# jiangzhengkai/mxdetection

Measured on AMD Instinct MI355X. Metric: images/sec (whole node) Faster R-CNN R50-FPN 3x800x1333, higher is better.
Workload: dtype bf16; 1 GPU; Faster R-CNN ResNet-50-FPN bf16 train step, batch 2/GPU, 3x800x1333 (padded 1344); global_batch=2, parallelism=dp1, frozen=stem+C2, frozen BN folded, optimizer=SGD momentum 0.9 wd 1e-4, launch=hipGraph replay, input=resident, wgrad_side_stream=True, rpn_branch_stream=True, grouped_wgrad=True, filter_prefetch_hints=True, params_trainable=41538304

## Files before the change

### include/mxdet.h

```cpp
#ifndef MXDET_H_
#define MXDET_H_

#include <stddef.h>
#include <stdint.h>

#ifdef __cplusplus
extern "C" {
#endif

#define MXDET_OK 0
#define MXDET_EINVAL (-1)
#define MXDET_ESHAPE (-2)
#define MXDET_EWORKSPACE (-3)
#define MXDET_EHIP (-4)
#define MXDET_ERCCL (-5)

#define MXDET_DTYPE_F32 0
#define MXDET_DTYPE_BF16 1

typedef void* mxdet_stream_t;

const char* mxdet_last_error(void);
const char* mxdet_version(void);

// ... 85 lines not shown
                         const int32_t* matched_gt, const float* gt_boxes, int32_t N, int32_t G_max, int64_t R,
                         int32_t num_classes, int32_t reg_dim, int32_t kind, float sigma, float std_x, float std_y,
                         float std_w, float std_h, float reg_weight, float* score, mxdet_stream_t stream);
size_t mxdet_ohem_select_workspace_bytes(int32_t N, int32_t P);
int mxdet_ohem_select(const float* score, const int32_t* labels, const float* rois, int32_t N, int32_t P, int32_t R,
                      float nms_thresh, int32_t* sel, int32_t* num_sel, int32_t* num_fg, void* workspace,
                      size_t workspace_bytes, mxdet_stream_t stream);
int mxdet_ohem_gather(const int32_t* sel, const float* pool_rois, const int32_t* pool_labels,
                      const int32_t* pool_matched_gt, const float* pool_bbox_targets, const float* pool_bbox_weights,
                      int32_t N, int32_t P, int32_t R, int32_t reg_dim, float* out_rois, int32_t* labels,
                      float* bbox_targets, float* bbox_weights, int32_t* matched_gt, mxdet_stream_t stream);

int mxdet_fpn_level_map(const float* rois, int64_t R, int32_t lvl_min, int32_t lvl_max,
                        int32_t* levels, mxdet_stream_t stream);
typedef struct {
  int32_t num_levels, lvl_min;
  int32_t H[8], W[8];
  float spatial_scale[8];
  void* feat[8];
} mxdet_feat_pyramid_t;
int mxdet_roi_align_fwd(const mxdet_feat_pyramid_t* f, int32_t N, int32_t C, const float* rois,
                        const int32_t* levels, int64_t R, int32_t PH, int32_t PW,
                        int32_t sampling_ratio, uint16_t* out, mxdet_stream_t stream);
int mxdet_roi_align_bwd(const mxdet_feat_pyramid_t* f, int32_t N, int32_t C, const float* rois,
                        const int32_t* levels, int64_t R, int32_t PH, int32_t PW,
                        int32_t sampling_ratio, const uint16_t* grad_out, mxdet_stream_t stream);
size_t mxdet_roi_align_bwd_gather_workspace_bytes(const mxdet_feat_pyramid_t* f, int32_t N, int64_t R);
int mxdet_roi_align_bwd_gather(const mxdet_feat_pyramid_t* f, int32_t N, int32_t C, const float* rois,
                               const int32_t* levels, int64_t R, int32_t PH, int32_t PW, int32_t sampling_ratio,
                               const uint16_t* grad_out, int32_t accumulate, void* workspace, size_t workspace_bytes,
                               mxdet_stream_t stream);
int mxdet_roi_align_bwd_gather_prepare(const mxdet_feat_pyramid_t* f, int32_t N, const float* rois,
                                       const int32_t* levels, int64_t R, int32_t PH, int32_t PW, int32_t sampling_ratio,
                                       void* workspace, size_t workspace_bytes, mxdet_stream_t stream);
int mxdet_roi_align_bwd_gather_prepared(const mxdet_feat_pyramid_t* f, int32_t N, int32_t C, const float* rois,
                                        const int32_t* levels, int64_t R, int32_t PH, int32_t PW, int32_t sampling_ratio,
                                        const uint16_t* grad_out, int32_t accumulate, void* workspace,
                                        size_t workspace_bytes, mxdet_stream_t stream);

typedef struct {
  mxdet_feat_pyramid_t pyr;
  int32_t N, C;
  int32_t PH, PW;
  int32_t sample_per_part;
  float trans_std;
  int32_t modulated;
// ... 376 lines not shown
```

### mxdetection_amd/_lib.py

```python
import ctypes as C
import os

_HERE = os.path.dirname(os.path.abspath(__file__))
LIB_PATH = os.environ.get("MXDET_LIB") or os.path.join(_HERE, "libmxdet_hip.so")

c_i32, c_i64, c_u32, c_f32, c_sz, c_vp = C.c_int32, C.c_int64, C.c_uint32, C.c_float, C.c_size_t, C.c_void_p


class PyramidT(C.Structure):
    _fields_ = [
        ("num_levels", c_i32), ("A", c_i32),
        ("H", c_i32 * 8), ("W", c_i32 * 8), ("stride", c_i32 * 8),
        ("cls", c_vp * 8), ("reg", c_vp * 8),
        ("cls_sn", c_i64 * 8), ("cls_sy", c_i64 * 8), ("cls_sx", c_i64 * 8), ("cls_sa", c_i64 * 8),
        ("reg_sn", c_i64 * 8), ("reg_sy", c_i64 * 8), ("reg_sx", c_i64 * 8), ("reg_sc", c_i64 * 8),
        ("dtype", c_i32), ("classes", c_i32),
        ("base_anchors", c_vp * 8),
    ]


class FeatPyramidT(C.Structure):
    _fields_ = [
        ("num_levels", c_i32), ("lvl_min", c_i32),
        ("H", c_i32 * 8), ("W", c_i32 * 8),
# ... 107 lines not shown
    "mxdet_proposal": (c_i32, [P(PyramidT), c_i32, c_vp, c_i32, c_i32, c_f32, c_f32, c_vp, c_vp, c_vp, c_vp,
                               c_vp, c_sz, c_vp]),
    "mxdet_anchor_target_workspace_bytes": (c_sz, [c_i32, c_i64, c_i32]),
    "mxdet_anchor_target": (c_i32, [c_vp, c_i64, c_vp, c_i32, c_i32, c_vp, c_f32, c_f32, c_f32, c_i32, c_f32,
                                    c_u32, c_u32, c_vp, c_u32, c_vp, c_vp, c_vp, c_vp, c_vp, c_sz, c_vp]),
    "mxdet_atss_assign_workspace_bytes": (c_sz, [c_i32, c_i64, c_i32]),
    "mxdet_atss_assign": (c_i32, [c_vp, c_i64, P(c_i64), c_i32, c_vp, c_i32, c_i32, c_i32, c_vp, c_vp, c_vp, c_vp, c_vp, c_sz,
                                  c_vp]),
    "mxdet_proposal_target": (c_i32, [c_vp, c_vp, c_i32, c_vp, c_i32, c_i32, c_i32, c_f32, c_f32, c_f32, c_f32,
                                      c_i32, c_i32, P(c_f32), P(c_f32), c_u32, c_u32, c_vp, c_u32, c_vp, c_vp, c_vp,
                                      c_vp, c_vp, c_vp, c_vp]),
    "mxdet_proposal_target_balanced": (c_i32, [c_vp, c_vp, c_i32, c_vp, c_i32, c_i32, c_i32, c_f32, c_f32, c_f32, c_f32,
                                               c_i32, c_i32, P(c_f32), P(c_f32), c_u32, c_u32, c_vp, c_u32, c_i32, c_vp, c_vp,
                                               c_vp, c_vp, c_vp, c_vp, c_vp]),
    "mxdet_ohem_roi_score": (c_i32, [c_vp, c_vp, c_i32, c_i32, c_i32, c_vp, c_vp, c_vp, c_vp, c_vp, c_vp, c_i32, c_i32, c_i64,
                                     c_i32, c_i32, c_i32, c_f32, c_f32, c_f32, c_f32, c_f32, c_f32, c_vp, c_vp]),
    "mxdet_ohem_select_workspace_bytes": (c_sz, [c_i32, c_i32]),
    "mxdet_ohem_select": (c_i32, [c_vp, c_vp, c_vp, c_i32, c_i32, c_i32, c_f32, c_vp, c_vp, c_vp, c_vp, c_sz, c_vp]),
    "mxdet_ohem_gather": (c_i32, [c_vp, c_vp, c_vp, c_vp, c_vp, c_vp, c_i32, c_i32, c_i32, c_i32, c_vp, c_vp, c_vp, c_vp,
                                  c_vp, c_vp]),
    "mxdet_fpn_level_map": (c_i32, [c_vp, c_i64, c_i32, c_i32, c_vp, c_vp]),
    "mxdet_roi_align_fwd": (c_i32, [P(FeatPyramidT), c_i32, c_i32, c_vp, c_vp, c_i64, c_i32, c_i32, c_i32, c_vp,
                                    c_vp]),
    "mxdet_roi_align_bwd": (c_i32, [P(FeatPyramidT), c_i32, c_i32, c_vp, c_vp, c_i64, c_i32, c_i32, c_i32, c_vp,
                                    c_vp]),
    "mxdet_roi_align_bwd_gather_workspace_bytes": (c_sz, [P(FeatPyramidT), c_i32, c_i64]),
    "mxdet_roi_align_bwd_gather": (c_i32, [P(FeatPyramidT), c_i32, c_i32, c_vp, c_vp, c_i64, c_i32, c_i32, c_i32, c_vp,
                                           c_i32, c_vp, c_sz, c_vp]),
    "mxdet_roi_align_bwd_gather_prepare": (c_i32, [P(FeatPyramidT), c_i32, c_vp, c_vp, c_i64, c_i32, c_i32, c_i32,
                                                   c_vp, c_sz, c_vp]),
    "mxdet_roi_align_bwd_gather_prepared": (c_i32, [P(FeatPyramidT), c_i32, c_i32, c_vp, c_vp, c_i64, c_i32, c_i32, c_i32,
                                                    c_vp, c_i32, c_vp, c_sz, c_vp]),
    "mxdet_smooth_l1_fwd": (c_i32, [c_vp, c_vp, c_vp, c_i64, c_f32, c_vp, c_vp]),
    "mxdet_smooth_l1_bwd": (c_i32, [c_vp, c_vp, c_vp, c_vp, c_i64, c_f32, c_i32, c_vp, c_vp]),
    "mxdet_loss_workspace_bytes": (c_sz, [c_i64]),
    "mxdet_focal_loss": (c_i32, [c_vp, c_i32, c_vp, c_i64, c_i32, c_f32, c_f32, c_f32, c_vp, c_vp, c_vp, c_sz,
                                 c_vp]),
    "mxdet_anchor_class_labels": (c_i32, [c_vp, c_vp, c_vp, c_i32, c_i64, c_i32, c_vp, c_vp, c_vp]),
    "mxdet_retina_loss_num_partials": (c_i32, [c_i32, c_i32, c_i32, c_i32]),
    "mxdet_retina_loss_level": (c_i32, [c_vp, c_vp, c_i32, c_i32, c_i32, c_i32, c_i32, c_i32, c_i32, c_vp, c_vp, c_i64,
                                        c_i64, c_f32, c_f32, c_f32, c_vp, c_f32, c_vp, c_vp, c_vp, c_vp]),
    "mxdet_rpn_loss_num_partials": (c_i32, [c_i32, c_i32, c_i32]),
    "mxdet_rpn_loss_level": (c_i32, [c_vp, c_i32, c_i32, c_i32, c_i32, c_i32, c_vp, c_vp, c_i64, c_i64, c_f32,
                                     c_f32, c_f32, c_vp, c_vp, c_vp]),
    "mxdet_loss_finalize": (c_i32, [c_vp, c_i32, c_i32, c_vp, c_vp]),
    "mxdet_rcnn_loss": (c_i32, [c_vp, c_vp, c_i32, c_i32, c_i32, c_vp, c_vp, c_vp, c_i64, c_i32, c_i32, c_f32,
# ... 168 lines not shown
```

### mxdetection_amd/csrc/roi_align.hip

```cpp
#include "roi_gather.h"

namespace mxdet {

struct RoiGeom {
  float start_w, start_h, bin_w, bin_h;
  int gh, gw, H, W, batch, lvl;
};

__device__ __forceinline__ RoiGeom roi_geom(const FeatPyr& f, const float* __restrict__ rois,
                                            const int32_t* __restrict__ levels, long long r, int PH,
                                            int PW, int sampling_ratio) {
  RoiGeom g;
  const float* q = rois + r * 5;
  roi_image_level(f, rois, levels, r, &g.lvl, &g.batch);
  const int l = g.lvl;
  float s = f.scale[l];
  g.start_w = q[1] * s;
  g.start_h = q[2] * s;
  float end_w = q[3] * s, end_h = q[4] * s;
  float rw = end_w - g.start_w, rh = end_h - g.start_h;
  rw = rw > 1.0f ? rw : 1.0f;
  rh = rh > 1.0f ? rh : 1.0f;
  g.bin_h = rh / (float)PH;
  g.bin_w = rw / (float)PW;
  if (sampling_ratio > 0) {
    g.gh = sampling_ratio;
    g.gw = sampling_ratio;
  } else {
    float ch = rh / (float)PH, cw = rw / (float)PW;
    int ih = (int)ch, iw = (int)cw;
    g.gh = ((float)ih < ch) ? ih + 1 : ih;
    g.gw = ((float)iw < cw) ? iw + 1 : iw;
  }
  g.H = f.H[l];
  g.W = f.W[l];
  return g;
}

struct Taps {
  int yl, yh, xl, xh;
  float w1, w2, w3, w4;
  bool valid;
};

__device__ __forceinline__ float roi_sample_coord(float start, float bin, int b, int i, int g) {
  float v = start + (float)b * bin;
  return v + (((float)i + 0.5f) * bin) / (float)g;
}

template <int SR>
__device__ __forceinline__ float roi_axis_coord(float start, float bin, int s, int sr) {
  const int b = SR ? s / SR : s / sr, i = s - b * (SR ? SR : sr);
  return roi_sample_coord(start, bin, b, i, SR ? SR : sr);
}

struct AxisSample { int lo, hi; float wlo, whi; bool valid; };

__device__ __forceinline__ AxisSample roi_axis_sample(float v, int L) {
  AxisSample a;
  a.valid = !(v < -1.0f || v > (float)L);
  if (v <= 0.0f) v = 0.0f;
  int lo = (int)v;
  if (lo >= L - 1) { a.hi = lo = L - 1; v = (float)lo; } else { a.hi = lo + 1; }
  a.lo = lo;
  a.whi = v - (float)lo;
  a.wlo = 1.0f - a.whi;
  return a;
}

__device__ __forceinline__ Taps bilinear_taps(float y, float x, int H, int W) {
  const AxisSample ay = roi_axis_sample(y, H), ax = roi_axis_sample(x, W);
  Taps t;
  t.valid = ay.valid && ax.valid;
  t.w1 = ay.wlo * ax.wlo; t.w2 = ay.wlo * ax.whi; t.w3 = ay.whi * ax.wlo; t.w4 = ay.whi * ax.whi;
  t.yl = ay.lo; t.yh = ay.hi; t.xl = ax.lo; t.xh = ax.hi;
  return t;
}

__global__ void __launch_bounds__(256)
roi_align_fwd_kernel(FeatPyr f, int C, const float* __restrict__ rois,
                     const int32_t* __restrict__ levels, int PH, int PW, int sampling_ratio,
                     uint16_t* __restrict__ out) {
  const long long r = blockIdx.x;
  const RoiGeom g = roi_geom(f, rois, levels, r, PH, PW, sampling_ratio);
  const int CG = C >> 3;
  const int items = PH * PW * CG;
  const uint16_t* feat = (const uint16_t*)f.feat[g.lvl] + (long long)g.batch * g.H * g.W * C;
  const float count = (float)(g.gh * g.gw);
  for (int it = threadIdx.x; it < items; it += blockDim.x) {
    int cg = it % CG;
    int bin = it / CG;
    int pw = bin % PW, ph = bin / PW;
    float acc[8];
#pragma unroll
    for (int k = 0; k < 8; ++k) acc[k] = 0.0f;
    for (int iy = 0; iy < g.gh; ++iy) {
      const float y = roi_sample_coord(g.start_h, g.bin_h, ph, iy, g.gh);
      for (int ix = 0; ix < g.gw; ++ix) {
        const float x = roi_sample_coord(g.start_w, g.bin_w, pw, ix, g.gw);
        const Taps t = bilinear_taps(y, x, g.H, g.W);
        if (!t.valid) continue;
        const uint4 v1 = *(const uint4*)(feat + ((long long)t.yl * g.W + t.xl) * C + cg * 8);
        const uint4 v2 = *(const uint4*)(feat + ((long long)t.yl * g.W + t.xh) * C + cg * 8);
        const uint4 v3 = *(const uint4*)(feat + ((long long)t.yh * g.W + t.xl) * C + cg * 8);
        const uint4 v4 = *(const uint4*)(feat + ((long long)t.yh * g.W + t.xh) * C + cg * 8);
        float a[8], b[8], c[8], d[8];
        unpack8_bf16(v1, a); unpack8_bf16(v2, b); unpack8_bf16(v3, c); unpack8_bf16(v4, d);
#pragma unroll
        for (int k = 0; k < 8; ++k) {
          float s = t.w1 * a[k];
          s = s + t.w2 * b[k];
          s = s + t.w3 * c[k];
          s = s + t.w4 * d[k];
          acc[k] = acc[k] + s;
        }
      }
    }
    uint32_t o[4];
#pragma unroll
    for (int k = 0; k < 4; ++k) {
      uint32_t lo = mxdet_f32_to_bf16(acc[2 * k] / count);
      uint32_t hi = mxdet_f32_to_bf16(acc[2 * k + 1] / count);
      o[k] = lo | (hi << 16);
    }
    *(uint4*)(out + (r * PH * PW + bin) * C + cg * 8) = make_uint4(o[0], o[1], o[2], o[3]);
  }
}

__global__ void __launch_bounds__(256)
roi_align_bwd_kernel(FeatPyr f, int C, const float* __restrict__ rois,
                     const int32_t* __restrict__ levels, int PH, int PW, int sampling_ratio,
                     const uint16_t* __restrict__ gout) {
  const long long r = blockIdx.x;
  const RoiGeom g = roi_geom(f, rois, levels, r, PH, PW, sampling_ratio);
  const int items = PH * PW * C;
  float* dfeat = (float*)f.feat[g.lvl] + (long long)g.batch * g.H * g.W * C;
  const float count = (float)(g.gh * g.gw);
// ... 182 lines not shown
          }
        }
      }
     }
    }
    if (accumulate && !touched) continue;
#pragma unroll
    for (int j = 0; j < kRoiTileW; ++j) {
      if (x0 + j >= W || !live) break;
      const float v[4] = {a0[j], a1[j], a2[j], a3[j]};
      seg_store4<true>(out + (size_t)j * C + c0, v, accumulate);
    }
  }
}

struct RoiSegGrid {
  int block0[9];
  int chunks[8];
  int segs_per_wg[8];
  int rows_per_wg[8];
  int bands[8];
};

struct RoiSeg {
  int nl;
  unsigned yy, xx;
  int r;
  float start_h, bin_h, start_w, bin_w;
};

typedef float f32x2_t __attribute__((ext_vector_type(2)));

__device__ __forceinline__ float lane_plus1(float v) {
  return __uint_as_float((unsigned)__builtin_amdgcn_update_dpp(0, (int)__float_as_uint(v), 0x101, 0xf, 0xf, true));
}

__device__ __forceinline__ void roi_axis_range(float start, float bin, int NS, int sr, int L, int* lo, int* hi) {
  int s0 = 0, s1 = NS - 1;
  while (s0 <= s1 && !roi_axis_sample(roi_axis_coord<0>(start, bin, s0, sr), L).valid) ++s0;
  while (s1 >= s0 && !roi_axis_sample(roi_axis_coord<0>(start, bin, s1, sr), L).valid) --s1;
  if (s0 > s1) { *lo = 1; *hi = 0; return; }
  *lo = roi_axis_sample(roi_axis_coord<0>(start, bin, s0, sr), L).lo;
  *hi = roi_axis_sample(roi_axis_coord<0>(start, bin, s1, sr), L).hi;
}

__global__ void __launch_bounds__(256)
roi_bwd_box_kernel(FeatPyr f, const float* __restrict__ rois, const int32_t* __restrict__ levels, int R, int PH, int PW,
                   int sr, RoiSeg* __restrict__ seg) {
  const int r = (int)(blockIdx.x * blockDim.x + threadIdx.x);
  if (r >= R) return;
  const RoiGeom g = roi_geom(f, rois, levels, r, PH, PW, sr);
  int ylo, yhi, xlo, xhi;
  roi_axis_range(g.start_h, g.bin_h, PH * sr, sr, g.H, &ylo, &yhi);
  roi_axis_range(g.start_w, g.bin_w, PW * sr, sr, g.W, &xlo, &xhi);
  RoiSeg o;
  const bool any = ylo <= yhi && xlo <= xhi;
  o.nl = g.batch | ((any ? g.lvl : 0xffff) << 16);
  o.yy = span_pack(ylo, yhi);
  o.xx = span_pack(xlo, xhi);
  o.r = r;
  o.start_h = g.start_h; o.bin_h = g.bin_h; o.start_w = g.start_w; o.bin_w = g.bin_w;
  seg[r] = o;
}

template <int PWT, int SR>
__global__ void __launch_bounds__(kSegWaves * 64)
roi_bwd_seg_kernel(FeatPyr f, RoiSegGrid gr, int C, const RoiSeg* __restrict__ seg, int R, int PH, int PW, int sr_,
                   const uint16_t* __restrict__ gout, int accumulate) {
  __shared__ unsigned e_xx[kSegChunk], e_yy[kSegChunk];
  __shared__ int e_r[kSegChunk];
  __shared__ float4 e_g[kSegChunk];
  __shared__ int wcnt[kSegWaves];
  __shared__ int s_cnt;
  const int sr = SR ? SR : sr_;
  const int tid = threadIdx.x, lane = tid & 63;
  const int wid = __builtin_amdgcn_readfirstlane(tid >> 6);
  const int bid = (int)blockIdx.x;
  const int l = level_of_block(gr.block0, f.num_levels, bid);
  const int rel = bid - gr.block0[l];
  const int per_img = gr.bands[l] * gr.chunks[l];
  const int n = rel / per_img, rem = rel - n * per_img;
  const int band = rem / gr.chunks[l], chunk = rem - band * gr.chunks[l];
  const int H = f.H[l], W = f.W[l];
  const int Y0 = band * gr.rows_per_wg[l];
  const int Y1 = (Y0 + gr.rows_per_wg[l] - 1 < H - 1) ? Y0 + gr.rows_per_wg[l] - 1 : H - 1;
// ... 133 lines not shown
      if (!live || (!multi_row && !last_round)) continue;
      const bool add = accumulate || (multi_row && !first_round);
      if (add && !touched) continue;
      uint16_t* out = (uint16_t*)f.feat[l] + ((size_t)(n * H + Y) * W + x0) * C + c0;
#pragma unroll
      for (int j = 0; j < kSegW; ++j) {
        if (x0 + j >= W) break;
        const float v[4] = {acc[j][0][0], acc[j][0][1], acc[j][1][0], acc[j][1][1]};
        seg_store4<true>(out + (size_t)j * C, v, add);
      }
    }
  }
}

static int fill(FeatPyr& d, const mxdet_feat_pyramid_t* f, int N, const char* who) {
  MXDET_REQUIRE(f != nullptr, MXDET_EINVAL, "%s: null pyramid", who);
  MXDET_REQUIRE(f->num_levels > 0 && f->num_levels <= 8, MXDET_ESHAPE, "%s: bad level count", who);
  for (int l = 0; l < f->num_levels; ++l)
    MXDET_REQUIRE(f->H[l] > 0 && f->W[l] > 0 && f->feat[l], MXDET_EINVAL, "%s: level %d incomplete", who, l);
  pyr_copy(d, *f, N);
  return MXDET_OK;
}

}

using namespace mxdet;

extern "C" int mxdet_roi_align_fwd(const mxdet_feat_pyramid_t* f, int32_t N, int32_t C,
                                   const float* rois, const int32_t* levels, int64_t R, int32_t PH,
                                   int32_t PW, int32_t sampling_ratio, uint16_t* out,
                                   mxdet_stream_t stream) {
  clear_error();
  FeatPyr d;
  int rc = fill(d, f, N, "roi_align_fwd");
  if (rc) return rc;
  MXDET_REQUIRE(N > 0 && C > 0 && (C % 8) == 0 && PH > 0 && PW > 0 && R >= 0, MXDET_ESHAPE,
                "roi_align_fwd: bad shape (C must be a multiple of 8)");
  if (R == 0) return MXDET_OK;
  MXDET_REQUIRE(rois && levels && out, MXDET_EINVAL, "roi_align_fwd: null pointer");
  hipLaunchKernelGGL(roi_align_fwd_kernel, dim3((unsigned)R), dim3(256), 0, as_stream(stream), d, C,
                     rois, levels, PH, PW, sampling_ratio, out);
  return check_launch("roi_align_fwd");
}

extern "C" int mxdet_roi_align_bwd(const mxdet_feat_pyramid_t* f, int32_t N, int32_t C,
                                   const float* rois, const int32_t* levels, int64_t R, int32_t PH,
                                   int32_t PW, int32_t sampling_ratio, const uint16_t* grad_out,
                                   mxdet_stream_t stream) {
  clear_error();
  FeatPyr d;
  int rc = fill(d, f, N, "roi_align_bwd");
  if (rc) return rc;
  MXDET_REQUIRE(N > 0 && C > 0 && PH > 0 && PW > 0 && R >= 0, MXDET_ESHAPE, "roi_align_bwd: bad shape");
  if (R == 0) return MXDET_OK;
  MXDET_REQUIRE(rois && levels && grad_out, MXDET_EINVAL, "roi_align_bwd: null pointer");
  hipLaunchKernelGGL(roi_align_bwd_kernel, dim3((unsigned)R), dim3(256), 0, as_stream(stream), d, C,
                     rois, levels, PH, PW, sampling_ratio, grad_out);
  return check_launch("roi_align_bwd");
}

static size_t roi_gather_carve(const FeatPyr& d, long long R, RoiRows* rr, size_t* off_tab, size_t* off_list, size_t* off_cnt,
                               size_t* off_box) {
  int rows_of[8], blocks_of[8];
  for (int l = 0; l < d.num_levels; ++l) {
// ... 2 lines not shown
    blocks_of[l] = rows_of[l] * rr->tiles_w[l];
  }
  const int rows = rr->rows_total = layout_block0(rr->row0, rows_of, d.num_levels);
  layout_block0(rr->block0, blocks_of, d.num_levels);
  size_t off = 0;
  *off_tab = off; off = align_up(off + (size_t)R * sizeof(RoiTab), 256);
  *off_list = off; off = align_up(off + (size_t)rows * (size_t)R * sizeof(unsigned short), 256);
  *off_cnt = off; off = align_up(off + (size_t)rows * sizeof(int), 256);
  *off_box = off; off = align_up(off + (size_t)R * sizeof(RoiBox), 256);
  return off;
}

extern "C" size_t mxdet_roi_align_bwd_gather_workspace_bytes(const mxdet_feat_pyramid_t* f, int32_t N, int64_t R) {
  if (!f || N <= 0 || R <= 0 || f->num_levels <= 0 || f->num_levels > 8) return 0;
  FeatPyr d;
  pyr_copy(d, *f, N);
  RoiRows rr; size_t a, b, c, e;
  return roi_gather_carve(d, R, &rr, &a, &b, &c, &e);
}

static int roi_bwd_gather_impl(const mxdet_feat_pyramid_t* f, int32_t N, int32_t C, const float* rois,
                               const int32_t* levels, int64_t R, int32_t PH, int32_t PW,
                               int32_t sampling_ratio, const uint16_t* grad_out, int32_t accumulate,
                               void* workspace, size_t workspace_bytes, mxdet_stream_t stream, int mode) {
  clear_error();
  FeatPyr d;
  int rc = fill(d, f, N, "roi_align_bwd_gather");
  if (rc) return rc;
  MXDET_REQUIRE(N > 0 && C > 0 && (C % 4) == 0 && PH > 0 && PW > 0 && R >= 0, MXDET_ESHAPE, "roi_align_bwd_gather: bad shape (C must be a multiple of 4)");
  MXDET_REQUIRE(sampling_ratio > 0 && PH * sampling_ratio <= kRoiMaxSamples && PW * sampling_ratio <= kRoiMaxSamples,
                MXDET_ESHAPE, "roi_align_bwd_gather: needs 0 < sampling_ratio and at most %d samples per axis", kRoiMaxSamples);
  MXDET_REQUIRE(R <= 65535, MXDET_ESHAPE, "roi_align_bwd_gather: at most 65535 rois");
  for (int l = 0; l < d.num_levels; ++l)
    MXDET_REQUIRE(d.H[l] < 32768 && d.W[l] < 32768, MXDET_ESHAPE, "roi_align_bwd_gather: level %d too large", l);
  MXDET_REQUIRE(rois && levels && (grad_out || mode == 1), MXDET_EINVAL, "roi_align_bwd_gather: null pointer");
  hipStream_t s = as_stream(stream);
  RoiRows rr; size_t o_tab, o_list, o_cnt, o_box;
  const size_t need = roi_gather_carve(d, R > 0 ? R : 1, &rr, &o_tab, &o_list, &o_cnt, &o_box);
  MXDET_REQUIRE(workspace && workspace_bytes >= need, MXDET_EWORKSPACE, "roi_align_bwd_gather: workspace %zu < %zu",
                workspace_bytes, need);
  if (PW <= 14 && R > 0 && tuning(MXDET_TUNE_ROI_TABLE) == 0) {
    static_assert(sizeof(RoiSeg) == sizeof(RoiBox), "the records live in the table form's box array");
    RoiSeg* seg = (RoiSeg*)((char*)workspace + o_box);
    RoiSegGrid gr;
    memset(&gr, 0, sizeof(gr));
    int blocks_of[8];
    const int rows_big = (int)tuning(MXDET_TUNE_ROI_ROWS);
    for (int l = 0; l < d.num_levels; ++l) {
      const int segs = ceil_div(d.W[l], kSegW);
      gr.chunks[l] = ceil_div(segs, kSegWaves);
      gr.segs_per_wg[l] = ceil_div(segs, gr.chunks[l]);
      gr.rows_per_wg[l] = (R > kSegChunk || d.H[l] < 64 || rows_big < 1) ? 1 : rows_big;
      gr.bands[l] = ceil_div(d.H[l], gr.rows_per_wg[l]);
      blocks_of[l] = d.N * gr.bands[l] * gr.chunks[l];
    }
    const int blocks = layout_block0(gr.block0, blocks_of, d.num_levels);
    if (mode != 2)
      hipLaunchKernelGGL(roi_bwd_box_kernel, dim3((unsigned)ceil_div((int)R, 256)), dim3(256), 0, s, d, rois, levels, (int)R,
                         PH, PW, sampling_ratio, seg);
    if (mode == 1) return check_launch("roi_align_bwd_gather_prepare");
    const dim3 grid((unsigned)blocks, (unsigned)ceil_div(C, 256));
#define MXDET_ROI_SEG(PWT, SR)                                                                                          \
  hipLaunchKernelGGL((roi_bwd_seg_kernel<PWT, SR>), grid, dim3(kSegWaves * 64), 0, s, d, gr, C, (const RoiSeg*)seg, (int)R, \
                     PH, PW, sampling_ratio, grad_out, accumulate)
    if (PW <= 7) { if (sampling_ratio == 2) MXDET_ROI_SEG(7, 2); else MXDET_ROI_SEG(7, 0); }
    else { if (sampling_ratio == 2) MXDET_ROI_SEG(14, 2); else MXDET_ROI_SEG(14, 0); }
#undef MXDET_ROI_SEG
    return check_launch("roi_align_bwd_gather");
  }
  if (mode == 1) return MXDET_OK;
  RoiTab* tab = (RoiTab*)((char*)workspace + o_tab);
  unsigned short* list = (unsigned short*)((char*)workspace + o_list);
  int* cnt = (int*)((char*)workspace + o_cnt);
  RoiBox* box = (RoiBox*)((char*)workspace + o_box);
  if (R > 0)
    hipLaunchKernelGGL(roi_bwd_tab_kernel, dim3((unsigned)R), dim3(64), 0, s, d, rois, levels, (long long)R, PH, PW,
                       sampling_ratio, tab, box);
  hipLaunchKernelGGL(roi_bwd_rows_kernel, dim3(rr.rows_total), dim3(64), 0, s, d, rr, (const RoiBox*)box,
                     (int)R, list, cnt);
  hipLaunchKernelGGL(roi_align_bwd_gather_kernel, dim3((unsigned)rr.block0[d.num_levels]), dim3(64), 0, s, d, rr, C,
                     (const RoiTab*)tab, (const RoiBox*)box, (int)R, (const unsigned short*)list, (const int*)cnt, PH, PW,
                     sampling_ratio, grad_out, accumulate);
  return check_launch("roi_align_bwd_gather");
}

extern "C" int mxdet_roi_align_bwd_gather(const mxdet_feat_pyramid_t* f, int32_t N, int32_t C, const float* rois,
                                          const int32_t* levels, int64_t R, int32_t PH, int32_t PW,
                                          int32_t sampling_ratio, const uint16_t* grad_out, int32_t accumulate,
                                          void* workspace, size_t workspace_bytes, mxdet_stream_t stream) {
  return roi_bwd_gather_impl(f, N, C, rois, levels, R, PH, PW, sampling_ratio, grad_out, accumulate, workspace,
                             workspace_bytes, stream, 0);
}

extern "C" int mxdet_roi_align_bwd_gather_prepare(const mxdet_feat_pyramid_t* f, int32_t N, const float* rois,
                                                  const int32_t* levels, int64_t R, int32_t PH, int32_t PW,
                                                  int32_t sampling_ratio, void* workspace, size_t workspace_bytes,
                                                  mxdet_stream_t stream) {
  return roi_bwd_gather_impl(f, N, 4, rois, levels, R, PH, PW, sampling_ratio, nullptr, 0, workspace, workspace_bytes,
                             stream, 1);
}

extern "C" int mxdet_roi_align_bwd_gather_prepared(const mxdet_feat_pyramid_t* f, int32_t N, int32_t C, const float* rois,
                                                   const int32_t* levels, int64_t R, int32_t PH, int32_t PW,
                                                   int32_t sampling_ratio, const uint16_t* grad_out, int32_t accumulate,
                                                   void* workspace, size_t workspace_bytes, mxdet_stream_t stream) {
  return roi_bwd_gather_impl(f, N, C, rois, levels, R, PH, PW, sampling_ratio, grad_out, accumulate, workspace,
                             workspace_bytes, stream, 2);
}
```

### mxdetection_amd/csrc/roi_gather.h

```cpp
#pragma once
#include "common.h"

namespace mxdet {

struct FeatPyr {
  int num_levels, lvl_min, N;
  int H[8], W[8];
  float scale[8];
  void* feat[8];
};

static inline void pyr_copy(FeatPyr& d, const mxdet_feat_pyramid_t& f, int N) {
  memset(&d, 0, sizeof(d));
  d.num_levels = f.num_levels;
  d.lvl_min = f.lvl_min;
  d.N = N;
  for (int l = 0; l < f.num_levels; ++l) {
    d.H[l] = f.H[l]; d.W[l] = f.W[l]; d.scale[l] = f.spatial_scale[l]; d.feat[l] = f.feat[l];
  }
}

__device__ __forceinline__ void roi_image_level(const FeatPyr& f, const float* __restrict__ rois,
                                                const int32_t* __restrict__ levels, long long r, int* lvl, int* n) {
  int l = levels[r] - f.lvl_min;
  *lvl = l < 0 ? 0 : (l >= f.num_levels ? f.num_levels - 1 : l);
  const int b = (int)rois[r * 5];
  *n = b < 0 ? 0 : (b >= f.N ? f.N - 1 : b);
}

static inline int layout_block0(int* block0, const int* per_level, int num_levels) {
  int blocks = 0;
  for (int l = 0; l < num_levels; ++l) {
    block0[l] = blocks;
    blocks += per_level[l];
  }
  block0[num_levels] = blocks;
  return blocks;
}

__device__ __forceinline__ int level_of_block(const int* block0, int num_levels, int bid) {
  int l = 0;
  while (l + 1 < num_levels && bid >= block0[l + 1]) ++l;
  return l;
}

constexpr unsigned kSpanEmpty = 0xffffu;
__device__ __forceinline__ unsigned span_pack(int lo, int hi) { return (unsigned)lo | ((unsigned)hi << 16); }
__device__ __forceinline__ int span_lo(unsigned packed) { return (int)(packed & 0xffffu); }
__device__ __forceinline__ int span_hi(unsigned packed) { return (int)(packed >> 16); }
__device__ __forceinline__ bool span_hits(unsigned packed, int lo, int hi) {
// ... 50 lines not shown
```

### mxdetection_amd/models/roi_extractors/fpn_roi_extractor.py

```python
import torch

from ...ops import dense
from ...ops.roi_align import (fpn_level_map, roi_align_backward, roi_align_backward_gather,
                              roi_align_backward_gather_prepare, roi_align_backward_gather_workspace, roi_align_forward)


class FPNRoIExtractor:
    def __init__(self, strides, pooled=(7, 7), sampling_ratio=2, lvl_min=2, device="cuda"):
        self.scales = [1.0 / s for s in strides]
        self.pooled, self.sr, self.lvl_min = pooled, sampling_ratio, lvl_min
        self.lvl_max = lvl_min + len(strides) - 1
        self.device = device
        self.out = None
        self.outs = {}
        self.dacc = None
        self.gather_ws = {}
        self.prepared = None

    def forward(self, feats, rois, prepare_gather=False):
        self.feats, self.rois = feats[:len(self.scales)], rois
        self.levels = fpn_level_map(rois, self.lvl_min, self.lvl_max)
        R, C = rois.shape[0], feats[0].shape[3]
        self.out = self.outs.setdefault((R, C), None)
        if self.out is None:
            self.out = torch.empty((R, self.pooled[0], self.pooled[1], C), dtype=torch.bfloat16, device=self.device)
            self.outs[(R, C)] = self.out
        self.prepared = None
        if prepare_gather:
            key = (R,) + tuple(tuple(f.shape[:3]) for f in self.feats)
            ws = self.gather_ws.get(key)
            if ws is None:
                ws = self.gather_ws[key] = roi_align_backward_gather_workspace(self.feats, self.scales, R, self.lvl_min)
            roi_align_backward_gather_prepare(self.feats, self.scales, rois, self.levels, self.pooled, self.sr,
                                              self.lvl_min, ws)
            self.prepared = ws
        return roi_align_forward(self.feats, self.scales, rois, self.levels, self.pooled, self.sr, self.lvl_min, self.out)

    def backward(self, grad_out, dP, shared_acc=None, zero=True, finalize=True):
        if shared_acc is not None:
            self.dacc = shared_acc
        if self.dacc is None:
            sizes = [f.numel() for f in self.feats]
            self.dacc_flat = torch.empty((sum(sizes),), dtype=torch.float32, device=self.device)
            self.dacc, off = [], 0
            for f, n in zip(self.feats, sizes):
                self.dacc.append(self.dacc_flat[off:off + n].view(f.shape))
                off += n
        if zero:
            if getattr(self, "dacc_flat", None) is not None:
                self.dacc_flat.zero_()
            else:
                for a in self.dacc:
                    a.zero_()
        roi_align_backward(self.dacc, self.scales, self.rois, self.levels, grad_out, self.sr, self.lvl_min)
        if finalize:
            self.finalize(dP)
        return self.dacc

# ... 15 lines not shown
```

### mxdetection_amd/ops/roi_align.py

```python
import ctypes as C

import torch

from .. import _lib
from .._lib import FeatPyramidT, check, ptr, stream_ptr


def fpn_level_map(rois, lvl_min=2, lvl_max=5):
    lib = _lib.load()
    R = rois.shape[0]
    levels = torch.empty((R,), dtype=torch.int32, device=rois.device)
    check(lib.mxdet_fpn_level_map(ptr(rois), R, lvl_min, lvl_max, ptr(levels), stream_ptr()), "fpn_level_map")
    return levels


def _pyr(feats, scales, lvl_min):
    d = FeatPyramidT()
    d.num_levels, d.lvl_min = len(feats), lvl_min
    for l, f in enumerate(feats):
        d.H[l], d.W[l] = f.shape[1], f.shape[2]
        d.spatial_scale[l] = scales[l]
        d.feat[l] = f.data_ptr()
    return d


def roi_align_forward(feats, scales, rois, levels, pooled=(7, 7), sampling_ratio=2, lvl_min=2, out=None):
    lib = _lib.load()
    N, C_ = feats[0].shape[0], feats[0].shape[3]
    R = rois.shape[0]
    if out is None:
        out = torch.empty((R, pooled[0], pooled[1], C_), dtype=torch.bfloat16, device=rois.device)
    d = _pyr(feats, scales, lvl_min)
    check(lib.mxdet_roi_align_fwd(C.byref(d), N, C_, ptr(rois), ptr(levels), R, pooled[0], pooled[1], sampling_ratio,
                                  ptr(out), stream_ptr()), "roi_align_fwd")
    return out


def roi_align_backward(dfeats, scales, rois, levels, grad_out, sampling_ratio=2, lvl_min=2):
    lib = _lib.load()
    N, C_ = dfeats[0].shape[0], dfeats[0].shape[3]
    R, PH, PW = grad_out.shape[0], grad_out.shape[1], grad_out.shape[2]
    d = _pyr(dfeats, scales, lvl_min)
    check(lib.mxdet_roi_align_bwd(C.byref(d), N, C_, ptr(rois), ptr(levels), R, PH, PW, sampling_ratio,
                                  ptr(grad_out), stream_ptr()), "roi_align_bwd")


_gather_ws = {}


def _gather_workspace(lib, d, N, R, device, workspace):
    need = lib.mxdet_roi_align_bwd_gather_workspace_bytes(C.byref(d), N, R)
    if workspace is None:
        key = (device, need)
        workspace = _gather_ws.get(key)
        if workspace is None:
            workspace = torch.empty((max(need, 256),), dtype=torch.uint8, device=device)
            _gather_ws[key] = workspace
    return workspace
# ... 30 lines not shown
```

Before: 457.3 images/sec.

## Fuse FPN level mapping and backward-gather prep into RoIAlign forward for training

Adds a training RoIAlign forward kernel that works out each RoI's FPN level inline, writes the levels array, and emits the backward-gather segment records from one thread per block. This replaces the separate fpn_level_map and gather-prepare launches. The forward kernel also gains a sampling_ratio=2 specialization that fully unrolls the four samples and issues all tap loads before accumulating, and its launch bounds now request higher occupancy. The cost is more registers per thread from the batched loads and a larger template kernel.

After: 459.6 images/sec (median of 6 runs). About the same (+0.5%).

```diff
diff --git a/include/mxdet.h b/include/mxdet.h
--- a/include/mxdet.h
+++ b/include/mxdet.h
@@ -131,6 +131,9 @@
 int mxdet_roi_align_fwd(const mxdet_feat_pyramid_t* f, int32_t N, int32_t C, const float* rois,
                         const int32_t* levels, int64_t R, int32_t PH, int32_t PW,
                         int32_t sampling_ratio, uint16_t* out, mxdet_stream_t stream);
+int mxdet_roi_align_fwd_train(const mxdet_feat_pyramid_t* f, int32_t N, int32_t C, const float* rois, int64_t R,
+                              int32_t PH, int32_t PW, int32_t sampling_ratio, uint16_t* out, int32_t* levels,
+                              void* workspace, size_t workspace_bytes, mxdet_stream_t stream);
 int mxdet_roi_align_bwd(const mxdet_feat_pyramid_t* f, int32_t N, int32_t C, const float* rois,
                         const int32_t* levels, int64_t R, int32_t PH, int32_t PW,
                         int32_t sampling_ratio, const uint16_t* grad_out, mxdet_stream_t stream);
diff --git a/mxdetection_amd/_lib.py b/mxdetection_amd/_lib.py
--- a/mxdetection_amd/_lib.py
+++ b/mxdetection_amd/_lib.py
@@ -153,6 +153,8 @@
     "mxdet_fpn_level_map": (c_i32, [c_vp, c_i64, c_i32, c_i32, c_vp, c_vp]),
     "mxdet_roi_align_fwd": (c_i32, [P(FeatPyramidT), c_i32, c_i32, c_vp, c_vp, c_i64, c_i32, c_i32, c_i32, c_vp,
                                     c_vp]),
+    "mxdet_roi_align_fwd_train": (c_i32, [P(FeatPyramidT), c_i32, c_i32, c_vp, c_i64, c_i32, c_i32, c_i32, c_vp, c_vp,
+                                          c_vp, c_sz, c_vp]),
     "mxdet_roi_align_bwd": (c_i32, [P(FeatPyramidT), c_i32, c_i32, c_vp, c_vp, c_i64, c_i32, c_i32, c_i32, c_vp,
                                     c_vp]),
     "mxdet_roi_align_bwd_gather_workspace_bytes": (c_sz, [P(FeatPyramidT), c_i32, c_i64]),
diff --git a/mxdetection_amd/csrc/roi_align.hip b/mxdetection_amd/csrc/roi_align.hip
--- a/mxdetection_amd/csrc/roi_align.hip
+++ b/mxdetection_amd/csrc/roi_align.hip
@@ -7,13 +7,12 @@
   int gh, gw, H, W, batch, lvl;
 };
 
-__device__ __forceinline__ RoiGeom roi_geom(const FeatPyr& f, const float* __restrict__ rois,
-                                            const int32_t* __restrict__ levels, long long r, int PH,
-                                            int PW, int sampling_ratio) {
+__device__ __forceinline__ RoiGeom roi_geom_on(const FeatPyr& f, const float* __restrict__ rois, long long r, int l,
+                                               int batch, int PH, int PW, int sampling_ratio) {
   RoiGeom g;
   const float* q = rois + r * 5;
-  roi_image_level(f, rois, levels, r, &g.lvl, &g.batch);
-  const int l = g.lvl;
+  g.lvl = l;
+  g.batch = batch;
   float s = f.scale[l];
   g.start_w = q[1] * s;
   g.start_h = q[2] * s;
@@ -37,6 +36,14 @@
   return g;
 }
 
+__device__ __forceinline__ RoiGeom roi_geom(const FeatPyr& f, const float* __restrict__ rois,
+                                            const int32_t* __restrict__ levels, long long r, int PH,
+                                            int PW, int sampling_ratio) {
+  int l, batch;
+  roi_image_level(f, rois, levels, r, &l, &batch);
+  return roi_geom_on(f, rois, r, l, batch, PH, PW, sampling_ratio);
+}
+
 struct Taps {
   int yl, yh, xl, xh;
   float w1, w2, w3, w4;
@@ -77,12 +84,56 @@
   return t;
 }
 
-__global__ void __launch_bounds__(256)
-roi_align_fwd_kernel(FeatPyr f, int C, const float* __restrict__ rois,
-                     const int32_t* __restrict__ levels, int PH, int PW, int sampling_ratio,
+struct RoiSeg {
+  int nl;
+  unsigned yy, xx;
+  int r;
+  float start_h, bin_h, start_w, bin_w;
+};
+
+__device__ __forceinline__ void roi_axis_range(float start, float bin, int NS, int sr, int L, int* lo, int* hi) {
+  int s0 = 0, s1 = NS - 1;
+  while (s0 <= s1 && !roi_axis_sample(roi_axis_coord<0>(start, bin, s0, sr), L).valid) ++s0;
+  while (s1 >= s0 && !roi_axis_sample(roi_axis_coord<0>(start, bin, s1, sr), L).valid) --s1;
+  if (s0 > s1) { *lo = 1; *hi = 0; return; }
+  *lo = roi_axis_sample(roi_axis_coord<0>(start, bin, s0, sr), L).lo;
+  *hi = roi_axis_sample(roi_axis_coord<0>(start, bin, s1, sr), L).hi;
+}
+
+__device__ __forceinline__ RoiSeg roi_seg_record(const RoiGeom& g, int r, int PH, int PW, int sr) {
+  int ylo, yhi, xlo, xhi;
+  roi_axis_range(g.start_h, g.bin_h, PH * sr, sr, g.H, &ylo, &yhi);
+  roi_axis_range(g.start_w, g.bin_w, PW * sr, sr, g.W, &xlo, &xhi);
+  RoiSeg o;
+  const bool any = ylo <= yhi && xlo <= xhi;
+  o.nl = g.batch | ((any ? g.lvl : 0xffff) << 16);
+  o.yy = span_pack(ylo, yhi);
+  o.xx = span_pack(xlo, xhi);
+  o.r = r;
+  o.start_h = g.start_h; o.bin_h = g.bin_h; o.start_w = g.start_w; o.bin_w = g.bin_w;
+  return o;
+}
+
+template <int SR, bool FUSED>
+__global__ void __launch_bounds__(256, 4)
+roi_align_fwd_kernel(FeatPyr f, int C, const float* __restrict__ rois, const int32_t* __restrict__ levels,
+                     int32_t* __restrict__ levels_out, RoiSeg* __restrict__ seg, int PH, int PW, int sampling_ratio,
                      uint16_t* __restrict__ out) {
   const long long r = blockIdx.x;
-  const RoiGeom g = roi_geom(f, rois, levels, r, PH, PW, sampling_ratio);
+  RoiGeom g;
+  if (FUSED) {
+    const float* q = rois + r * 5;
+    const int lvl_max = f.lvl_min + f.num_levels - 1;
+    int k = mxdet_fpn_level(q[1], q[2], q[3], q[4]);
+    k = k < f.lvl_min ? f.lvl_min : (k > lvl_max ? lvl_max : k);
+    g = roi_geom_on(f, rois, r, k - f.lvl_min, roi_image(f, rois, r), PH, PW, SR ? SR : sampling_ratio);
+    if (threadIdx.x == blockDim.x - 1) {
+      levels_out[r] = k;
+      if (seg) seg[r] = roi_seg_record(g, (int)r, PH, PW, SR ? SR : sampling_ratio);
+    }
+  } else {
+    g = roi_geom(f, rois, levels, r, PH, PW, SR ? SR : sampling_ratio);
+  }
   const int CG = C >> 3;
   const int items = PH * PW * CG;
   const uint16_t* feat = (const uint16_t*)f.feat[g.lvl] + (long long)g.batch * g.H * g.W * C;
@@ -94,25 +145,58 @@
     float acc[8];
 #pragma unroll
     for (int k = 0; k < 8; ++k) acc[k] = 0.0f;
-    for (int iy = 0; iy < g.gh; ++iy) {
-      const float y = roi_sample_coord(g.start_h, g.bin_h, ph, iy, g.gh);
-      for (int ix = 0; ix < g.gw; ++ix) {
-        const float x = roi_sample_coord(g.start_w, g.bin_w, pw, ix, g.gw);
-        const Taps t = bilinear_taps(y, x, g.H, g.W);
-        if (!t.valid) continue;
-        const uint4 v1 = *(const uint4*)(feat + ((long long)t.yl * g.W + t.xl) * C + cg * 8);
-        const uint4 v2 = *(const uint4*)(feat + ((long long)t.yl * g.W + t.xh) * C + cg * 8);
-        const uint4 v3 = *(const uint4*)(feat + ((long long)t.yh * g.W + t.xl) * C + cg * 8);
-        const uint4 v4 = *(const uint4*)(feat + ((long long)t.yh * g.W + t.xh) * C + cg * 8);
+    if (SR) {
+      constexpr int NS = SR ? SR * SR : 1;
+      Taps t[NS];
+#pragma unroll
+      for (int iy = 0; iy < SR; ++iy) {
+        const float y = roi_sample_coord(g.start_h, g.bin_h, ph, iy, SR);
+#pragma unroll
+        for (int ix = 0; ix < SR; ++ix)
+          t[iy * SR + ix] = bilinear_taps(y, roi_sample_coord(g.start_w, g.bin_w, pw, ix, SR), g.H, g.W);
+      }
+      uint4 v[NS][4];
+#pragma unroll
+      for (int s = 0; s < NS; ++s) {
+        v[s][0] = *(const uint4*)(feat + ((long long)t[s].yl * g.W + t[s].xl) * C + cg * 8);
+        v[s][1] = *(const uint4*)(feat + ((long long)t[s].yl * g.W + t[s].xh) * C + cg * 8);
+        v[s][2] = *(const uint4*)(feat + ((long long)t[s].yh * g.W + t[s].xl) * C + cg * 8);
+        v[s][3] = *(const uint4*)(feat + ((long long)t[s].yh * g.W + t[s].xh) * C + cg * 8);
+      }
+#pragma unroll
+      for (int s = 0; s < NS; ++s) {
         float a[8], b[8], c[8], d[8];
-        unpack8_bf16(v1, a); unpack8_bf16(v2, b); unpack8_bf16(v3, c); unpack8_bf16(v4, d);
+        unpack8_bf16(v[s][0], a); unpack8_bf16(v[s][1], b); unpack8_bf16(v[s][2], c); unpack8_bf16(v[s][3], d);
 #pragma unroll
         for (int k = 0; k < 8; ++k) {
-          float s = t.w1 * a[k];
-          s = s + t.w2 * b[k];
-          s = s + t.w3 * c[k];
-          s = s + t.w4 * d[k];
-          acc[k] = acc[k] + s;
+          float u = t[s].w1 * a[k];
+          u = u + t[s].w2 * b[k];
+          u = u + t[s].w3 * c[k];
+          u = u + t[s].w4 * d[k];
+          acc[k] = t[s].valid ? acc[k] + u : acc[k];
+        }
+      }
+    } else {
+      for (int iy = 0; iy < g.gh; ++iy) {
+        const float y = roi_sample_coord(g.start_h, g.bin_h, ph, iy, g.gh);
+        for (int ix = 0; ix < g.gw; ++ix) {
+          const float x = roi_sample_coord(g.start_w, g.bin_w, pw, ix, g.gw);
+          const Taps t = bilinear_taps(y, x, g.H, g.W);
+          if (!t.valid) continue;
+          const uint4 v1 = *(const uint4*)(feat + ((long long)t.yl * g.W + t.xl) * C + cg * 8);
+          const uint4 v2 = *(const uint4*)(feat + ((long long)t.yl * g.W + t.xh) * C + cg * 8);
+          const uint4 v3 = *(const uint4*)(feat + ((long long)t.yh * g.W + t.xl) * C + cg * 8);
+          const uint4 v4 = *(const uint4*)(feat + ((long long)t.yh * g.W + t.xh) * C + cg * 8);
+          float a[8], b[8], c[8], d[8];
+          unpack8_bf16(v1, a); unpack8_bf16(v2, b); unpack8_bf16(v3, c); unpack8_bf16(v4, d);
+#pragma unroll
+          for (int k = 0; k < 8; ++k) {
+            float s = t.w1 * a[k];
+            s = s + t.w2 * b[k];
+            s = s + t.w3 * c[k];
+            s = s + t.w4 * d[k];
+            acc[k] = acc[k] + s;
+          }
         }
       }
     }
@@ -341,26 +425,10 @@
   int bands[8];
 };
 
-struct RoiSeg {
-  int nl;
-  unsigned yy, xx;
-  int r;
-  float start_h, bin_h, start_w, bin_w;
-};
-
 typedef float f32x2_t __attribute__((ext_vector_type(2)));
 
 __device__ __forceinline__ float lane_plus1(float v) {
   return __uint_as_float((unsigned)__builtin_amdgcn_update_dpp(0, (int)__float_as_uint(v), 0x101, 0xf, 0xf, true));
-}
-
-__device__ __forceinline__ void roi_axis_range(float start, float bin, int NS, int sr, int L, int* lo, int* hi) {
-  int s0 = 0, s1 = NS - 1;
-  while (s0 <= s1 && !roi_axis_sample(roi_axis_coord<0>(start, bin, s0, sr), L).valid) ++s0;
-  while (s1 >= s0 && !roi_axis_sample(roi_axis_coord<0>(start, bin, s1, sr), L).valid) --s1;
-  if (s0 > s1) { *lo = 1; *hi = 0; return; }
-  *lo = roi_axis_sample(roi_axis_coord<0>(start, bin, s0, sr), L).lo;
-  *hi = roi_axis_sample(roi_axis_coord<0>(start, bin, s1, sr), L).hi;
 }
 
 __global__ void __launch_bounds__(256)
@@ -368,18 +436,7 @@
                    int sr, RoiSeg* __restrict__ seg) {
   const int r = (int)(blockIdx.x * blockDim.x + threadIdx.x);
   if (r >= R) return;
-  const RoiGeom g = roi_geom(f, rois, levels, r, PH, PW, sr);
-  int ylo, yhi, xlo, xhi;
-  roi_axis_range(g.start_h, g.bin_h, PH * sr, sr, g.H, &ylo, &yhi);
-  roi_axis_range(g.start_w, g.bin_w, PW * sr, sr, g.W, &xlo, &xhi);
-  RoiSeg o;
-  const bool any = ylo <= yhi && xlo <= xhi;
-  o.nl = g.batch | ((any ? g.lvl : 0xffff) << 16);
-  o.yy = span_pack(ylo, yhi);
-  o.xx = span_pack(xlo, xhi);
-  o.r = r;
-  o.start_h = g.start_h; o.bin_h = g.bin_h; o.start_w = g.start_w; o.bin_w = g.bin_w;
-  seg[r] = o;
+  seg[r] = roi_seg_record(roi_geom(f, rois, levels, r, PH, PW, sr), r, PH, PW, sr);
 }
 
 template <int PWT, int SR>
@@ -559,6 +616,17 @@
   return MXDET_OK;
 }
 
+template <bool FUSED>
+static void roi_fwd_launch(const FeatPyr& d, int C, const float* rois, const int32_t* levels, int32_t* levels_out,
+                           RoiSeg* seg, int64_t R, int PH, int PW, int sampling_ratio, uint16_t* out, hipStream_t s) {
+  if (sampling_ratio == 2)
+    hipLaunchKernelGGL((roi_align_fwd_kernel<2, FUSED>), dim3((unsigned)R), dim3(256), 0, s, d, C, rois, levels, levels_out,
+                       seg, PH, PW, sampling_ratio, out);
+  else
+    hipLaunchKernelGGL((roi_align_fwd_kernel<0, FUSED>), dim3((unsigned)R), dim3(256), 0, s, d, C, rois, levels, levels_out,
+                       seg, PH, PW, sampling_ratio, out);
+}
+
 }
 
 using namespace mxdet;
@@ -575,8 +643,7 @@
                 "roi_align_fwd: bad shape (C must be a multiple of 8)");
   if (R == 0) return MXDET_OK;
   MXDET_REQUIRE(rois && levels && out, MXDET_EINVAL, "roi_align_fwd: null pointer");
-  hipLaunchKernelGGL(roi_align_fwd_kernel, dim3((unsigned)R), dim3(256), 0, as_stream(stream), d, C,
-                     rois, levels, PH, PW, sampling_ratio, out);
+  roi_fwd_launch<false>(d, C, rois, levels, nullptr, nullptr, R, PH, PW, sampling_ratio, out, as_stream(stream));
   return check_launch("roi_align_fwd");
 }
 
@@ -625,7 +692,8 @@
 static int roi_bwd_gather_impl(const mxdet_feat_pyramid_t* f, int32_t N, int32_t C, const float* rois,
                                const int32_t* levels, int64_t R, int32_t PH, int32_t PW,
                                int32_t sampling_ratio, const uint16_t* grad_out, int32_t accumulate,
-                               void* workspace, size_t workspace_bytes, mxdet_stream_t stream, int mode) {
+                               void* workspace, size_t workspace_bytes, mxdet_stream_t stream, int mode,
+                               RoiSeg** records = nullptr) {
   clear_error();
   FeatPyr d;
   int rc = fill(d, f, N, "roi_align_bwd_gather");
@@ -636,7 +704,7 @@
   MXDET_REQUIRE(R <= 65535, MXDET_ESHAPE, "roi_align_bwd_gather: at most 65535 rois");
   for (int l = 0; l < d.num_levels; ++l)
     MXDET_REQUIRE(d.H[l] < 32768 && d.W[l] < 32768, MXDET_ESHAPE, "roi_align_bwd_gather: level %d too large", l);
-  MXDET_REQUIRE(rois && levels && (grad_out || mode == 1), MXDET_EINVAL, "roi_align_bwd_gather: null pointer");
+  MXDET_REQUIRE(rois && levels && (grad_out || mode == 1 || mode == 3), MXDET_EINVAL, "roi_align_bwd_gather: null pointer");
   hipStream_t s = as_stream(stream);
   RoiRows rr; size_t o_tab, o_list, o_cnt, o_box;
   const size_t need = roi_gather_carve(d, R > 0 ? R : 1, &rr, &o_tab, &o_list, &o_cnt, &o_box);
@@ -645,6 +713,7 @@
   if (PW <= 14 && R > 0 && tuning(MXDET_TUNE_ROI_TABLE) == 0) {
     static_assert(sizeof(RoiSeg) == sizeof(RoiBox), "the records live in the table form's box array");
     RoiSeg* seg = (RoiSeg*)((char*)workspace + o_box);
+    if (mode == 3) { *records = seg; return MXDET_OK; }
     RoiSegGrid gr;
     memset(&gr, 0, sizeof(gr));
     int blocks_of[8];
@@ -671,7 +740,7 @@
 #undef MXDET_ROI_SEG
     return check_launch("roi_align_bwd_gather");
   }
-  if (mode == 1) return MXDET_OK;
+  if (mode == 1 || mode == 3) return MXDET_OK;
   RoiTab* tab = (RoiTab*)((char*)workspace + o_tab);
   unsigned short* list = (unsigned short*)((char*)workspace + o_list);
   int* cnt = (int*)((char*)workspace + o_cnt);
@@ -710,3 +779,24 @@
   return roi_bwd_gather_impl(f, N, C, rois, levels, R, PH, PW, sampling_ratio, grad_out, accumulate, workspace,
                              workspace_bytes, stream, 2);
 }
+
+extern "C" int mxdet_roi_align_fwd_train(const mxdet_feat_pyramid_t* f, int32_t N, int32_t C, const float* rois, int64_t R,
+                                         int32_t PH, int32_t PW, int32_t sampling_ratio, uint16_t* out, int32_t* levels,
+                                         void* workspace, size_t workspace_bytes, mxdet_stream_t stream) {
+  clear_error();
+  FeatPyr d;
+  int rc = fill(d, f, N, "roi_align_fwd_train");
+  if (rc) return rc;
+  MXDET_REQUIRE(N > 0 && C > 0 && (C % 8) == 0 && PH > 0 && PW > 0 && R >= 0, MXDET_ESHAPE,
+                "roi_align_fwd_train: bad shape (C must be a multiple of 8)");
+  if (R == 0) return MXDET_OK;
+  MXDET_REQUIRE(rois && levels && out, MXDET_EINVAL, "roi_align_fwd_train: null pointer");
+  RoiSeg* seg = nullptr;
+  if (workspace) {
+    rc = roi_bwd_gather_impl(f, N, C, rois, levels, R, PH, PW, sampling_ratio, nullptr, 0, workspace, workspace_bytes,
+                             stream, 3, &seg);
+    if (rc) return rc;
+  }
+  roi_fwd_launch<true>(d, C, rois, nullptr, levels, seg, R, PH, PW, sampling_ratio, out, as_stream(stream));
+  return check_launch("roi_align_fwd_train");
+}
diff --git a/mxdetection_amd/csrc/roi_gather.h b/mxdetection_amd/csrc/roi_gather.h
--- a/mxdetection_amd/csrc/roi_gather.h
+++ b/mxdetection_amd/csrc/roi_gather.h
@@ -20,12 +20,16 @@
   }
 }
 
+__device__ __forceinline__ int roi_image(const FeatPyr& f, const float* __restrict__ rois, long long r) {
+  const int b = (int)rois[r * 5];
+  return b < 0 ? 0 : (b >= f.N ? f.N - 1 : b);
+}
+
 __device__ __forceinline__ void roi_image_level(const FeatPyr& f, const float* __restrict__ rois,
                                                 const int32_t* __restrict__ levels, long long r, int* lvl, int* n) {
   int l = levels[r] - f.lvl_min;
   *lvl = l < 0 ? 0 : (l >= f.num_levels ? f.num_levels - 1 : l);
-  const int b = (int)rois[r * 5];
-  *n = b < 0 ? 0 : (b >= f.N ? f.N - 1 : b);
+  *n = roi_image(f, rois, r);
 }
 
 static inline int layout_block0(int* block0, const int* per_level, int num_levels) {
diff --git a/mxdetection_amd/models/roi_extractors/fpn_roi_extractor.py b/mxdetection_amd/models/roi_extractors/fpn_roi_extractor.py
--- a/mxdetection_amd/models/roi_extractors/fpn_roi_extractor.py
+++ b/mxdetection_amd/models/roi_extractors/fpn_roi_extractor.py
@@ -2,7 +2,7 @@
 
 from ...ops import dense
 from ...ops.roi_align import (fpn_level_map, roi_align_backward, roi_align_backward_gather,
-                              roi_align_backward_gather_prepare, roi_align_backward_gather_workspace, roi_align_forward)
+                              roi_align_backward_gather_workspace, roi_align_forward, roi_align_forward_train)
 
 
 class FPNRoIExtractor:
@@ -19,7 +19,6 @@
 
     def forward(self, feats, rois, prepare_gather=False):
         self.feats, self.rois = feats[:len(self.scales)], rois
-        self.levels = fpn_level_map(rois, self.lvl_min, self.lvl_max)
         R, C = rois.shape[0], feats[0].shape[3]
         self.out = self.outs.setdefault((R, C), None)
         if self.out is None:
@@ -31,9 +30,11 @@
             ws = self.gather_ws.get(key)
             if ws is None:
                 ws = self.gather_ws[key] = roi_align_backward_gather_workspace(self.feats, self.scales, R, self.lvl_min)
-            roi_align_backward_gather_prepare(self.feats, self.scales, rois, self.levels, self.pooled, self.sr,
-                                              self.lvl_min, ws)
+            _, self.levels = roi_align_forward_train(self.feats, self.scales, rois, self.pooled, self.sr, self.lvl_min,
+                                                     self.out, workspace=ws)
             self.prepared = ws
+            return self.out
+        self.levels = fpn_level_map(rois, self.lvl_min, self.lvl_max)
         return roi_align_forward(self.feats, self.scales, rois, self.levels, self.pooled, self.sr, self.lvl_min, self.out)
 
     def backward(self, grad_out, dP, shared_acc=None, zero=True, finalize=True):
diff --git a/mxdetection_amd/ops/roi_align.py b/mxdetection_amd/ops/roi_align.py
--- a/mxdetection_amd/ops/roi_align.py
+++ b/mxdetection_amd/ops/roi_align.py
@@ -34,6 +34,22 @@
     check(lib.mxdet_roi_align_fwd(C.byref(d), N, C_, ptr(rois), ptr(levels), R, pooled[0], pooled[1], sampling_ratio,
                                   ptr(out), stream_ptr()), "roi_align_fwd")
     return out
+
+
+def roi_align_forward_train(feats, scales, rois, pooled=(7, 7), sampling_ratio=2, lvl_min=2, out=None, levels=None,
+                            workspace=None):
+    lib = _lib.load()
+    N, C_ = feats[0].shape[0], feats[0].shape[3]
+    R = rois.shape[0]
+    if out is None:
+        out = torch.empty((R, pooled[0], pooled[1], C_), dtype=torch.bfloat16, device=rois.device)
+    if levels is None:
+        levels = torch.empty((R,), dtype=torch.int32, device=rois.device)
+    d = _pyr(feats, scales, lvl_min)
+    check(lib.mxdet_roi_align_fwd_train(C.byref(d), N, C_, ptr(rois), R, pooled[0], pooled[1], sampling_ratio, ptr(out),
+                                        ptr(levels), ptr(workspace), 0 if workspace is None else workspace.numel(),
+                                        stream_ptr()), "roi_align_fwd_train")
+    return out, levels
 
 
 def roi_align_backward(dfeats, scales, rois, levels, grad_out, sampling_ratio=2, lvl_min=2):
```
